# chaofengc/FeMaSR

Measured on AMD Instinct MI355X. Metric: SR output megapixels/sec at x4 (128->512), higher is better.
Workload: dtype f32 (1x1 convs / nn.Linear: every fp32 operand split EXACTLY into three bf16 terms, six partial products, fp32 accumulation on the bf16 matrix pipe - closer to fp64 than the fp32 fmaf chain, bit-identical to the CPU oracle)

## Files before the change

femasr_amd/_lib.py:

```python
import ctypes
import os

_HERE = os.path.dirname(os.path.abspath(__file__))
SO_PATH = os.path.join(_HERE, 'csrc', 'libfemasr_hip.so')

c_int, c_i64, c_f32 = ctypes.c_int, ctypes.c_int64, ctypes.c_float
vp, szt = ctypes.c_void_p, ctypes.c_size_t


class FemasrError(RuntimeError):
    pass


MAX_CODEBOOKS = 3


class Config(ctypes.Structure):
    _fields_ = ([(n, ctypes.c_int32) for n in ('in_channel', 'gt_resolution', 'lq_stage', 'scale_factor', 'use_quantize',
                                               'use_residual', 'n_codebooks')] +
                [(n, ctypes.c_int32 * MAX_CODEBOOKS) for n in ('codebook_scale', 'n_e', 'e_dim')] +
                [('device', ctypes.c_int32)])


class ConvArgs(ctypes.Structure):
# ... 119 lines not shown
    'femasr_channels_merge_u8': (c_int, [vp, vp, vp, vp, c_int, c_int, c_int, c_int, vp, vp, c_int, vp, vp, c_int, vp]),
    'femasr_clock_probe': (c_int, [vp, c_int, vp]),
    'femasr_clock_probe_entries': (c_int, []),
}
ENCODE_SIGNATURES = {
    'femasr_encode_workspace_bytes': (c_int, [vp, c_int, c_int, c_int, c_int, ctypes.POINTER(szt)]),
    'femasr_encode': (c_int, [vp, vp, vp, c_int, c_int, c_int, c_int, c_int, c_int, vp, vp, szt]),
    'femasr_index_histogram_workspace_bytes': (c_int, [c_int, c_i64, c_int, ctypes.POINTER(szt)]),
    'femasr_index_histogram': (c_int, [vp, vp, c_int, c_i64, c_int, vp, vp, vp, szt]),
}
RESAMPLE_SIGNATURES = {
    'femasr_resample_u8': (c_int, [vp, vp, c_int, c_int, c_int, vp, c_int, c_int, vp, vp, c_int, vp, vp, c_int]),
    'femasr_resample_tile': (c_int, []),
}
JPEG_SIGNATURES = {
    'femasr_jpeg_coefficients_u8': (c_int, [vp, c_int, c_int, c_int, c_int, vp, vp, vp, vp, vp, vp]),
    'femasr_jpeg_entropy_rows': (ctypes.c_longlong, [vp, vp, vp, c_int, c_int, c_int, c_int, c_int, c_int, vp, szt]),
    'femasr_jpeg_entropy_bound': (szt, [c_int, c_int, c_int, c_int]),
}
c_u64 = ctypes.c_uint64
DEGRADE_SIGNATURES = {
    'femasr_degrade_blur_f32': (c_int, [vp, vp, c_int, c_int, vp, c_int, c_int, vp]),
    'femasr_degrade_resize_f32': (c_int, [vp, vp, c_int, c_int, vp, c_int, c_int, vp, vp, c_int, vp, vp, c_int, vp, vp]),
    'femasr_degrade_noise_f32': (c_int, [vp, vp, vp, ctypes.c_longlong, c_u64, c_int, ctypes.POINTER(ctypes.c_double), c_u64]),
    'femasr_degrade_quantize_u8': (c_int, [vp, vp, vp, ctypes.c_longlong]),
    'femasr_degrade_unit_f32': (c_int, [vp, vp, c_int, c_int, c_int, vp]),
    'femasr_jpeg_decode_u8': (c_int, [vp, vp, vp, vp, c_int, c_int, c_int, c_int, vp, vp, vp, c_int]),
}
DEBUG_SIGNATURES = {
    'femasr_debug_set_wino_limits': (c_int, [vp, c_int, c_int]),
    'femasr_debug_mfma_bf16': (c_int, [vp, vp, vp, vp, c_int, vp]),
    'femasr_gemm_force_config': (c_int, [c_int]),
    'femasr_conv_small_launch_blocks': (c_int, [c_int]),
    'femasr_debug_conv_variant_name': (c_int, [ctypes.POINTER(ConvArgs), ctypes.c_char_p, c_int]),
    'femasr_debug_weight_image_bytes': (c_int, [vp, c_int, ctypes.POINTER(szt)]),
    'femasr_debug_math_eval': (c_int, [vp, c_int, vp, ctypes.c_longlong, vp]),
}

_lib = None


def load():
    global _lib
    if _lib is not None:
        return _lib
    if not os.path.exists(SO_PATH):
        raise FemasrError(
            f'{SO_PATH} not found: the HIP extension is not built. Run `python femasr_amd/csrc/build.py` '
            '(needs hipcc; cross-compiles gfx950 without a GPU). There is no CPU fallback.')
    lib = ctypes.CDLL(SO_PATH)
    lib.femasr_version.restype = c_int
    if lib.femasr_version() != ABI_VERSION:
        raise FemasrError(f'{SO_PATH} reports ABI version {lib.femasr_version()}, this binding is written for {ABI_VERSION} '
                          '(femasr_conv_args layout): rebuild with `python femasr_amd/csrc/build.py --force`')
    for name, (res, args) in list(SIGNATURES.items()) + list(ENCODE_SIGNATURES.items()) + list(RESAMPLE_SIGNATURES.items()) + list(JPEG_SIGNATURES.items()) + list(DEGRADE_SIGNATURES.items()) + list(DEBUG_SIGNATURES.items()):
        fn = getattr(lib, name)
        fn.restype = res
        fn.argtypes = args
    _lib = lib
    return lib


def check(rc):
    if rc != 0:
        msg = load().femasr_last_error()
        raise FemasrError(f'libfemasr_hip error {rc}: {msg.decode() if msg else "?"}')
# ... 5 lines not shown
```

femasr_amd/csrc/gemm_common.h:

```cpp
#pragma once
#include "conv_common.h"
#include "detmath.h"
#include <stdlib.h>

typedef float f32x16 __attribute__((ext_vector_type(16)));

namespace {

struct GemmParams {
    const float *A;
    const void *W;
    const float *bias, *res1, *res2;
    float *out;
    int M, N, K, MB, NB, NT32;
};

struct GemmFrame {
    int t, lane, wave, wm, wn;
    int nb, mb, m0, n0;
    int h, c31;

    __device__ __forceinline__ GemmFrame(int MB, int NB, int bt)
    {
        t = threadIdx.x, lane = t & 63;
        wave = __builtin_amdgcn_readfirstlane(t >> 6);
        wm = wave >> 1, wn = wave & 1;
        const int L = xcd_remap(blockIdx.x, MB * NB);
        nb = L % NB, mb = L / NB;
        m0 = mb * bt, n0 = nb * bt;
        h = lane >> 5, c31 = lane & 31;
    }
};

template <int WT, int ACT, int NRES, bool NULL_BIAS, class Elem>
__device__ __forceinline__ void gemm_store_epilogue(const GemmParams &p, const GemmFrame &f, float *lds, Elem elem)
{
    const int m0 = f.m0, n0 = f.n0, wm = f.wm, wn = f.wn, h = f.h, c31 = f.c31;
    float *T = lds + f.wave * TSCRATCH;
    const int trow = f.lane >> 3, tq = f.lane & 7;
    const float *ra = p.res1 ? p.res1 : p.res2, *rb = (p.res1 && p.res2) ? p.res2 : nullptr;
    const bool vec = (p.N & 3) == 0;
    f32x4_t r1[4] = {}, r2[4] = {};
    auto fetch_bias = [&](int j) {
        const int col = n0 + (wn * WT + j) * 32 + 4 * tq;
        f32x4_t b4 = {0.f, 0.f, 0.f, 0.f};
        if (!NULL_BIAS || p.bias) b4 = *reinterpret_cast<const f32x4_t *>(p.bias + (col < p.N ? col : 0));
        return b4;
    };
    auto fetch_res = [&](int tl) {
        if (NRES == 0 || !vec) return;
        const int rbase = m0 + (wm * WT + tl / WT) * 32, col = n0 + (wn * WT + tl % WT) * 32 + 4 * tq;
#pragma unroll
        for (int k = 0; k < 4; ++k) {
            const int row = rbase + trow + 8 * k;
            const size_t o = (col < p.N && row < p.M) ? (size_t)row * p.N + col : 0;
            r1[k] = *reinterpret_cast<const f32x4_t *>(ra + o);
            if (NRES >= 2) r2[k] = *reinterpret_cast<const f32x4_t *>(rb + o);
        }
    };
#pragma unroll
    for (int tl = 0; tl < WT * WT; ++tl) {
        const int i = tl / WT, j = tl % WT;
        const int rbase = m0 + (wm * WT + i) * 32, cbase = n0 + (wn * WT + j) * 32;
// ... 41 lines not shown
struct FragItem {
    int lane, n, k0;
    size_t tile;
};
__device__ __forceinline__ FragItem frag_item(size_t item, int NT32)
{
    const int lane = (int)(item & 63);
    const size_t tile = item >> 6;
    const int nt = (int)(tile % NT32), st = (int)(tile / NT32);
    return {lane, 32 * nt + (lane & 31), 16 * st + 8 * (lane >> 5), tile};
}

template <class Params>
struct GemmVariant {
    const char *name;
    void (*kern)(const Params);
    int lds;
    unsigned long long attr_devs;
};

inline int gemm_params(const femasr_conv_args *a, const char *who, int Ho, int Wo, int K, GemmParams &p)
{
    FEMASR_REQUIRE(a->act == FEMASR_ACT_NONE || a->act == FEMASR_ACT_GELU, "%s: bad activation %d", who, a->act);
    const long long M = (long long)a->B * Ho * Wo;
    FEMASR_REQUIRE(a->Ho == Ho && a->Wo == Wo, "%s: Ho/Wo mismatch", who);
    FEMASR_REQUIRE(M > 0 && M < (1ll << 31) - 256, "%s: bad row count", who);
    p.A = a->in; p.bias = a->bias; p.res1 = a->res1; p.res2 = a->res2; p.out = a->out;
    p.M = (int)M; p.N = a->Cout; p.K = K;
    p.NT32 = (p.N + 31) / 32;
    return FEMASR_OK;
}

template <class Params, int N>
int gemm_variant_launch(hipStream_t s, GemmVariant<Params> (&table)[N], int vi, int bt, Params &p, int *variant_out, double *flops_out)
{
    GemmVariant<Params> &v = table[vi];
    p.MB = (p.M + bt - 1) / bt; p.NB = (p.N + bt - 1) / bt;
    FEMASR_CHECK(femasr_allow_dynamic_lds((const void *)v.kern, &v.attr_devs, (size_t)v.lds));
    hipLaunchKernelGGL(v.kern, dim3((unsigned)(p.MB * p.NB)), dim3(256), (size_t)v.lds, s, p);
    FEMASR_CHECK_HIP(hipGetLastError());
    if (variant_out) *variant_out = vi;
    if (flops_out) *flops_out = 2.0 * (double)p.M * (double)p.N * (double)p.K;
    return FEMASR_OK;
}

}
```

femasr_amd/csrc/kernel_meta.py:

```python
import functools
import os
import re
import struct
import subprocess
import sys
import tempfile

HERE = os.path.dirname(os.path.abspath(__file__))
READELF = '/opt/rocm/lib/llvm/bin/llvm-readelf'
ALLOW_SCRATCH = (
    'conv3x3_halo_bf16x3_kernel',
)


def device_elf(obj_path):
    data = open(obj_path, 'rb').read()
    i = data.find(b'__CLANG_OFFLOAD_BUNDLE__')
    if i < 0:
        return None
    n = struct.unpack_from('<Q', data, i + 24)[0]
    off = i + 32
    for _ in range(n):
        o, sz, tl = struct.unpack_from('<QQQ', data, off)
        off += 24
# ... 97 lines not shown
    for line in txt.splitlines():
        m = re.match(r'^[0-9a-f]+ <(\S+)>:', line)
        if m:
            cur = out.setdefault(m.group(1), [])
            continue
        m = re.match(r'^\s+(\S+)\s*(.*?)\s*//\s*([0-9A-Fa-f]+):', line)
        if m and cur is not None:
            cur.append((int(m.group(3), 16), m.group(1), m.group(2)))
    return out


def mfma_loops(insts):
    addr_index = {a: i for i, (a, _, _) in enumerate(insts)}
    loops = []
    for i, (a, op, args) in enumerate(insts):
        if not op.startswith('s_cbranch') and op != 's_branch':
            continue
        try:
            simm = int(args.split()[0])
        except (ValueError, IndexError):
            continue
        if simm >= 32768:
            simm -= 65536
        if simm >= 0:
            continue
        tgt = addr_index.get(a + 4 + 4 * simm)
        if tgt is None:
            continue
        if any(o.startswith('v_mfma') for _, o, _ in insts[tgt:i]):
            loops.append((tgt, i))
    return [l for l in loops if not any(m != l and l[0] <= m[0] and m[1] <= l[1] for m in loops)]


def check_counted_waits(obj=None):
    obj = obj or os.path.join(HERE, 'kernels_gemm_bf16.o')
    problems = []
    src = open(os.path.join(HERE, 'kernels_gemm_bf16.hip')).read()
    src_counts = sorted({int(v) for v in re.findall(r's_waitcnt vmcnt\((\d+)\)', src)})
    want_counts = sorted({0} | set(COUNTED['vmcnt']))
    if src_counts != want_counts:
        problems.append(f'kernels_gemm_bf16.hip waits for vmcnt {src_counts}, kernel_meta.COUNTED expects {want_counts}: update both together')
    seen = 0
    for name, insts in disassemble(obj).items():
        if 'gemm_bf16s_kernel' not in name:
            continue
        seen += 1
        want = COUNTED
        loops = mfma_loops(insts)
        if len(loops) != want['loops']:
            problems.append(f'{demangle_short(name)}: expected {want["loops"]} MFMA loop(s), found {len(loops)}')
            continue
        for lo, hi in loops:
            body = insts[lo:hi + 1]
            vmem, waits = {}, {}
            for _, op, args in body:
                if op.startswith(VMEM_PREFIXES):
                    vmem[op] = vmem.get(op, 0) + 1
                if op == 's_waitcnt':
                    for n in re.findall(r'vmcnt\((\d+)\)', args):
                        waits[int(n)] = waits.get(int(n), 0) + 1
            want_vmem = {k: v for k, v in want.items() if k not in ('vmcnt', 'loops')}
            if vmem != want_vmem:
                problems.append(f'{demangle_short(name)}: VMEM instructions in the MFMA loop {vmem}, the counted waits assume exactly {want_vmem}')
            if waits != want['vmcnt']:
                problems.append(f'{demangle_short(name)}: vmcnt waits in the MFMA loop {waits}, the source has {want["vmcnt"]}')
            if not any(op == 's_barrier' for _, op, _ in body):
                problems.append(f'{demangle_short(name)}: no s_barrier in the MFMA loop')
    if seen < N_GEMM_BF16S:
        problems.append(f'only {seen} gemm_bf16s_kernel instantiations found in {obj}')
    return problems


META = ('vgpr_count', 'agpr_count', 'sgpr_count', 'vgpr_spill_count', 'sgpr_spill_count', 'private_segment_fixed_size', 'group_segment_fixed_size')


def code_of(csrc, objs=None):
    meta = {(r['file'], r['name']): tuple(r.get(k) for k in META) for r in kernels(csrc) if objs is None or r['file'] in objs}
    return {f: {n: ([i[1:] for i in insts], meta[f, n]) for n, insts in disassemble(os.path.join(csrc, f)).items() if (f, n) in meta}
            for f in sorted({f for f, _ in meta})}


def diff(here, there, rename=()):
    ren = dict(rename)
    old = {f: {ren.get(n, n): v for n, v in ks.items()} for f, ks in there.items()}
    lines = [(f, n, 'same' if v == old[f][n] else 'differs') for f, ks in here.items() for n, v in ks.items() if n in old.get(f, {})]
    lone_here = [(f, n) for f, ks in here.items() for n in ks if n not in old.get(f, {})]
    lone_there = [(g, n) for g, ks in old.items() for n in ks if n not in here.get(g, {})]
    for f, n in lone_here:
        homes = [g for g, m in lone_there if m == n]
        if len(homes) == 1:
            lone_there.remove((homes[0], n))
            lines.append((f + ' < ' + homes[0], n, 'same' if here[f][n] == old[homes[0]][n] else 'differs'))
        else:
            lines.append((f, n, 'only here'))
    return sorted(lines + [(g, n, 'only there') for g, n in lone_there])


LOOP_PREFIXES = VMEM_PREFIXES + ('ds_', 'v_mfma', 's_waitcnt', 's_barrier')


# ... 41 lines not shown
```

femasr_amd/csrc/kernels_gemm_bf16.hip:

```cpp
#include "gemm_common.h"

typedef __bf16 bf16x8 __attribute__((ext_vector_type(8)));
typedef __bf16 bf16x2_t __attribute__((ext_vector_type(2)));
typedef float f32x2_t __attribute__((ext_vector_type(2)));

namespace {

struct GemmSParams : GemmParams {
    int imH, imW, Cin, tapmul;
    int imHo, imWo, stride;
};

__device__ float g_gs_zero_page[64];

constexpr int GS_A_HALF = 3 * 2 * 128;
constexpr int GS_A_BYTES = 2 * GS_A_HALF * 16;
constexpr int GS_W_STAGE = 4 * 3 * 64;
constexpr int GS_W_STAGES = 4;
constexpr int GS_LDS_BYTES = GS_A_BYTES + GS_W_STAGES * GS_W_STAGE * 16;
static_assert(4 * TSCRATCH * 4 <= GS_LDS_BYTES, "epilogue scratch overlays the main-loop buffers");

__device__ __forceinline__ unsigned cvt_pk_bf16(float a, float b)
{
    const bf16x2_t r = __builtin_convertvector(f32x2_t{a, b}, bf16x2_t);
    return __builtin_bit_cast(unsigned, r);
}

__device__ __forceinline__ void split3_pair(float a, float b, unsigned &p1, unsigned &p2, unsigned &p3)
{
    p1 = cvt_pk_bf16(a, b);
    const float ra = a - __uint_as_float(p1 << 16), rb = b - __uint_as_float(p1 & 0xffff0000u);
    p2 = cvt_pk_bf16(ra, rb);
    const float sa = ra - __uint_as_float(p2 << 16), sb = rb - __uint_as_float(p2 & 0xffff0000u);
    p3 = cvt_pk_bf16(sa, sb);
}
__device__ __forceinline__ void split3_x8(const f32x4_t &u, const f32x4_t &v, uint4 &q1, uint4 &q2, uint4 &q3)
{
    split3_pair(u[0], u[1], q1.x, q2.x, q3.x);
    split3_pair(u[2], u[3], q1.y, q2.y, q3.y);
    split3_pair(v[0], v[1], q1.z, q2.z, q3.z);
    split3_pair(v[2], v[3], q1.w, q2.w, q3.w);
}

typedef __attribute__((address_space(3))) void *lds_vptr_s;

__device__ __forceinline__ void dma3(const uint4 *w, unsigned d0)
{
    unsigned m0_keep;
    asm volatile("s_mov_b32 %0, m0\n\t"
                 "s_mov_b32 m0, %1\n\ts_nop 0\n\tglobal_load_lds_dwordx4 %4, off\n\t"
                 "s_mov_b32 m0, %2\n\ts_nop 0\n\tglobal_load_lds_dwordx4 %5, off\n\t"
                 "s_mov_b32 m0, %3\n\ts_nop 0\n\tglobal_load_lds_dwordx4 %6, off\n\t"
                 "s_mov_b32 m0, %0"
                 : "=&s"(m0_keep) : "s"(d0), "s"(d0 + 1024u), "s"(d0 + 2048u), "v"(w), "v"(w + 64), "v"(w + 128) : "memory");
}

template <int ACT, int NRES, int CONV>
__global__ __launch_bounds__(256, 2) void gemm_bf16s_kernel(const GemmSParams p)
{
    extern __shared__ __attribute__((aligned(16))) unsigned char smem_raw[];
    uint4 *S = reinterpret_cast<uint4 *>(smem_raw);

    const GemmFrame f(p.MB, p.NB, 128);
    const int t = f.t, lane = f.lane, wave = f.wave, wm = f.wm, wn = f.wn, m0 = f.m0, n0 = f.n0, h = f.h, c31 = f.c31;
    const int nsteps = p.K >> 4;

    int ntile = (n0 >> 5) + wave;
    ntile = ntile < p.NT32 ? ntile : p.NT32 - 1;
    const uint4 *srcW = static_cast<const uint4 *>(p.W) + (size_t)ntile * 192 + lane;
    const size_t wstep = (size_t)p.NT32 * 192;
    const unsigned lds0 = __builtin_amdgcn_readfirstlane((unsigned)(size_t)(lds_vptr_s)S);

    f32x16 hi[2][2], lo[2][2];
#pragma unroll
    for (int i = 0; i < 2; ++i)
#pragma unroll
        for (int j = 0; j < 2; ++j)
#pragma unroll
            for (int r = 0; r < 16; ++r) { hi[i][j][r] = 0.f; lo[i][j][r] = 0.f; }

    auto compute = [&](const uint4 *As, const int (&aoff)[2], const uint4 *Ws) {
        bf16x8 fa[3][2], fb[3][2];
        constexpr int order[3] = {2, 0, 1};
#pragma unroll
        for (int q = 0; q < 3; ++q) {
            const int pa = order[q], pb = q == 0 ? 0 : (q == 1 ? 2 : 1);
#pragma unroll
            for (int rt = 0; rt < 2; ++rt) fa[pa][rt] = __builtin_bit_cast(bf16x8, As[pa * 256 + aoff[rt]]);
#pragma unroll
            for (int ct = 0; ct < 2; ++ct) fb[pb][ct] = __builtin_bit_cast(bf16x8, Ws[ct * 192 + pb * 64]);
        }
#define GS_TERM(ACC, PA, PB)                                                                                       \
    _Pragma("unroll") for (int rt = 0; rt < 2; ++rt)                                                              \
        _Pragma("unroll") for (int ct = 0; ct < 2; ++ct)                                                          \
            ACC[rt][ct] = __builtin_amdgcn_mfma_f32_32x32x16_bf16(fa[PA][rt], fb[PB][ct], ACC[rt][ct], 0, 0, 0);
        GS_TERM(lo, 2, 0)
        GS_TERM(lo, 0, 2)
        GS_TERM(lo, 1, 1)
        GS_TERM(lo, 1, 0)
        GS_TERM(lo, 0, 1)
        GS_TERM(hi, 0, 0)
#undef GS_TERM
    };
    const int boff = (wn * 2) * 192 + lane;

    {
        uint4 *Al = S;
        uint4 *Wl = reinterpret_cast<uint4 *>(smem_raw + GS_A_BYTES);
        const int g2 = t & 1, srow = t >> 1;
        int grow = m0 + srow;
        grow = grow < p.M ? grow : p.M - 1;
        const float *srcA = p.A + (size_t)grow * p.K + 8 * g2;
        unsigned tapmask = 0;
        if (CONV) {
            const int ox = grow % p.imWo, oy = (grow / p.imWo) % p.imHo, n = grow / (p.imWo * p.imHo);
            const int px = ox * p.stride, py = oy * p.stride;
            srcA = p.A + (((size_t)n * p.imH + py) * p.imW + px) * p.Cin + 8 * g2;
#pragma unroll
            for (int tp = 0; tp < 9; ++tp) {
                const int yy = py + tp / 3 - 1, xx = px + tp % 3 - 1;
                tapmask |= (yy >= 0 && yy < p.imH && xx >= 0 && xx < p.imW ? 1u : 0u) << tp;
            }
        }
        const int cpc = p.Cin >> 5;
        const int dstA = g2 * 128 + ((srow + 4 * g2) & 127);
        f32x4_t ar[2][4] = {};
        const int nch = p.K >> 5;
        auto loadA = [&](int c, f32x4_t (&r)[4]) {
            const int cl = c < nch ? c : nch - 1;
            const float *q;
            if (CONV) {
                const int tap = (cl * p.tapmul) >> 20, cc = cl - tap * cpc;
                const int ky = (tap * 11) >> 5, kx = tap - 3 * ky;
                const int off = ((ky - 1) * p.imW + (kx - 1)) * p.Cin + cc * 32;
                q = ((tapmask >> tap) & 1u) ? srcA + off : g_gs_zero_page + 8 * g2;
            } else {
                q = srcA + cl * 32;
            }
            asm volatile("global_load_dwordx4 %0, %4, off\n\tglobal_load_dwordx4 %1, %4, off offset:16\n\t"
                         "global_load_dwordx4 %2, %4, off offset:64\n\tglobal_load_dwordx4 %3, %4, off offset:80"
                         : "=&v"(r[0]), "=&v"(r[1]), "=&v"(r[2]), "=&v"(r[3]) : "v"(q) : "memory");
        };
        const unsigned ldsW = lds0 + (unsigned)GS_A_BYTES + (unsigned)wave * 3072u;
        auto issueW = [&](int s) {
            dma3(srcW + (size_t)(s < nsteps ? s : nsteps - 1) * wstep, ldsW + (unsigned)(s & (GS_W_STAGES - 1)) * (GS_W_STAGE * 16));
        };
        auto splitA = [&](const f32x4_t &u, const f32x4_t &v, int half) {
            uint4 q1, q2, q3;
            split3_x8(u, v, q1, q2, q3);
            uint4 *d = Al + half * GS_A_HALF + dstA;
            d[0] = q1;
            d[256] = q2;
            d[512] = q3;
        };
        int aoff[2];
#pragma unroll
        for (int rt = 0; rt < 2; ++rt) {
            const int row = wm * 64 + rt * 32 + c31;
            aoff[rt] = h * 128 + ((row + 4 * h) & 127);
        }
        auto step = [&](int s) { compute(Al + (s & 1) * GS_A_HALF, aoff, Wl + (s & (GS_W_STAGES - 1)) * GS_W_STAGE + boff); };
        issueW(0);
        loadA(0, ar[0]);
        issueW(1);
        issueW(2);
        loadA(1, ar[1]);
        asm volatile("s_waitcnt vmcnt(10)" : "+v"(ar[0][0]), "+v"(ar[0][1]), "+v"(ar[0][2]), "+v"(ar[0][3]) :: "memory");
        splitA(ar[0][0], ar[0][1], 0);

        auto chunk = [&](int c, f32x4_t (&cur)[4], f32x4_t (&nxt)[4]) {
            asm volatile("s_waitcnt vmcnt(14)\n\ts_waitcnt lgkmcnt(0)" ::: "memory");
            __builtin_amdgcn_s_barrier();
            asm volatile("" ::: "memory");
            issueW(2 * c + 3);
            splitA(cur[2], cur[3], 1);
            step(2 * c);
            asm volatile("s_waitcnt vmcnt(10)\n\ts_waitcnt lgkmcnt(0)" ::: "memory");
            __builtin_amdgcn_s_barrier();
            asm volatile("" ::: "memory");
            issueW(2 * c + 4);
            loadA(c + 2, cur);
            asm volatile("s_waitcnt vmcnt(10)" : "+v"(nxt[0]), "+v"(nxt[1]), "+v"(nxt[2]), "+v"(nxt[3]) :: "memory");
            splitA(nxt[0], nxt[1], 0);
            step(2 * c + 1);
        };
#pragma unroll 1
        for (int c = 0; c < nch; c += 2) {
            chunk(c, ar[0], ar[1]);
            chunk(c + 1, ar[1], ar[0]);
        }
    }

    asm volatile("s_waitcnt vmcnt(0)" ::: "memory");
    float *T = reinterpret_cast<float *>(smem_raw) + wave * TSCRATCH;
    {
        const int trow = lane >> 3, tq = lane & 7;
        const float *ra = p.res1 ? p.res1 : p.res2, *rb = (p.res1 && p.res2) ? p.res2 : nullptr;
        const bool vec = (p.N & 3) == 0;
        f32x4_t bpre[2] = {}, r1[2][4] = {}, r2[2][4] = {};
        auto fetch_res = [&](int tl, f32x4_t (&d1)[4], f32x4_t (&d2)[4]) {
            if (NRES == 0 || !vec) return;
            const int rbase = m0 + (wm * 2 + (tl >> 1)) * 32, col = n0 + (wn * 2 + (tl & 1)) * 32 + 4 * tq;
#pragma unroll
            for (int k = 0; k < 4; ++k) {
                const int row = rbase + trow + 8 * k;
                const size_t o = (col < p.N && row < p.M) ? (size_t)row * p.N + col : 0;
                d1[k] = *reinterpret_cast<const f32x4_t *>(ra + o);
                if (NRES >= 2) d2[k] = *reinterpret_cast<const f32x4_t *>(rb + o);
            }
        };
        if (vec) {
#pragma unroll
            for (int j = 0; j < 2; ++j) {
                const int col = n0 + (wn * 2 + j) * 32 + 4 * tq;
                bpre[j] = *reinterpret_cast<const f32x4_t *>(p.bias + (col < p.N ? col : 0));
            }
        }
        fetch_res(0, r1[0], r2[0]);
        asm volatile("s_waitcnt lgkmcnt(0)" ::: "memory");
        __builtin_amdgcn_s_barrier();
        asm volatile("" ::: "memory");
#pragma unroll
        for (int tl = 0; tl < 4; ++tl) {
            const int i = tl >> 1, j = tl & 1;
            const int rbase = m0 + (wm * 2 + i) * 32, cbase = n0 + (wn * 2 + j) * 32;
            if (vec) {
                const int col = cbase + 4 * tq;
                const bool cok = col < p.N;
                if (tl + 1 < 4) fetch_res(tl + 1, r1[(tl + 1) & 1], r2[(tl + 1) & 1]);
#pragma unroll
                for (int r = 0; r < 16; ++r) T[((r & 3) + 8 * (r >> 2) + 4 * h) * TPITCH + c31] = hi[i][j][r] + lo[i][j][r];
                const f32x4_t b4 = bpre[j];
#pragma unroll
                for (int k = 0; k < 4; ++k) {
                    const f32x4_t a4 = *reinterpret_cast<const f32x4_t *>(T + (trow + 8 * k) * TPITCH + 4 * tq);
                    float v[4] = {a4[0] + b4[0], a4[1] + b4[1], a4[2] + b4[2], a4[3] + b4[3]};
                    if (ACT == FEMASR_ACT_GELU) {
                        const det_f32x2 g0 = det_gelu2(det_f32x2{v[0], v[1]}), g1 = det_gelu2(det_f32x2{v[2], v[3]});
                        v[0] = g0[0]; v[1] = g0[1]; v[2] = g1[0]; v[3] = g1[1];
                    }
#pragma unroll
                    for (int e = 0; e < 4; ++e) {
                        if (NRES >= 1) v[e] = v[e] + r1[tl & 1][k][e];
                        if (NRES >= 2) v[e] = v[e] + r2[tl & 1][k][e];
                    }
                    const int row = rbase + trow + 8 * k;
                    if (cok && row < p.M) *reinterpret_cast<f32x4_t *>(p.out + (size_t)row * p.N + col) = f32x4_t{v[0], v[1], v[2], v[3]};
                }
            } else {
                const int col = cbase + c31;
#pragma unroll
                for (int r = 0; r < 16; ++r) {
                    const int row = rbase + (r & 3) + 8 * (r >> 2) + 4 * h;
                    if (row < p.M && col < p.N) {
                        const size_t o = (size_t)row * p.N + col;
                        float v = (hi[i][j][r] + lo[i][j][r]) + p.bias[col];
                        if (ACT == FEMASR_ACT_GELU) v = det_gelu(v);
                        if (NRES >= 1) v = v + ra[o];
                        if (NRES >= 2) v = v + rb[o];
                        p.out[o] = v;
                    }
                }
            }
        }
    }
}

struct GatherOI {
    static __device__ __forceinline__ void load(const float *in, int I, int n, int k0, f32x4_t &u, f32x4_t &v)
    {
        u = *reinterpret_cast<const f32x4_t *>(in + (size_t)n * I + k0);
        v = *reinterpret_cast<const f32x4_t *>(in + (size_t)n * I + k0 + 4);
    }
};
struct GatherOIHW3x3 {
    static __device__ __forceinline__ void load(const float *in, int I, int n, int k0, f32x4_t &u, f32x4_t &v)
    {
        const int tap = k0 / I, c0 = k0 - tap * I;
        float w[8];
#pragma unroll
        for (int j = 0; j < 8; ++j) w[j] = in[((size_t)n * I + c0 + j) * 9 + tap];
        u = f32x4_t{w[0], w[1], w[2], w[3]};
        v = f32x4_t{w[4], w[5], w[6], w[7]};
    }
};
template <class GATHER>
__global__ void repack_bf16s_kernel(const float *__restrict__ in, int O, int I, uint4 *__restrict__ out, size_t total)
{
    const int NT32 = (O + 31) / 32;
    for (size_t i = blockIdx.x * (size_t)blockDim.x + threadIdx.x; i < total; i += (size_t)gridDim.x * blockDim.x) {
        const FragItem it = frag_item(i, NT32);
        f32x4_t u = {0.f, 0.f, 0.f, 0.f}, v = {0.f, 0.f, 0.f, 0.f};
        if (it.n < O) GATHER::load(in, I, it.n, it.k0, u, v);
        uint4 q1, q2, q3;
        split3_x8(u, v, q1, q2, q3);
        uint4 *o = out + it.tile * 192 + it.lane;
        o[0] = q1;
        o[64] = q2;
        o[128] = q3;
    }
}

__global__ void mfma_bf16_probe_kernel(const unsigned short *__restrict__ a, const unsigned short *__restrict__ b, const float *__restrict__ c,
                                       int N, float *__restrict__ d)
{
    const int lane = threadIdx.x, i = lane & 31, h = lane >> 5;
    const int n = blockIdx.x * 32 + i;
    union { bf16x8 v; unsigned short u[8]; } fa, fb;
#pragma unroll
    for (int e = 0; e < 8; ++e) { fa.u[e] = n < N ? a[(size_t)n * 16 + 8 * h + e] : 0; fb.u[e] = n < N ? b[(size_t)n * 16 + 8 * h + e] : 0; }
    f32x16 acc;
#pragma unroll
    for (int r = 0; r < 16; ++r) acc[r] = ((r & 3) + 8 * (r >> 2) + 4 * h == i && n < N) ? c[n] : 0.f;
    acc = __builtin_amdgcn_mfma_f32_32x32x16_bf16(fa.v, fb.v, acc, 0, 0, 0);
#pragma unroll
    for (int r = 0; r < 16; ++r)
        if ((r & 3) + 8 * (r >> 2) + 4 * h == i && n < N) d[n] = acc[r];
}

#define GS_VARIANT(ACT, NRES) { "gemm_bf16s<act=" #ACT ",nres=" #NRES ">", gemm_bf16s_kernel<ACT, NRES, 0>, GS_LDS_BYTES, 0ull }
#define GC_VARIANT(NRES) { "conv3x3_bf16s<128px x128,9Cin split GEMM,nres=" #NRES ">", gemm_bf16s_kernel<0, NRES, 1>, GS_LDS_BYTES, 0ull }
GemmVariant<GemmSParams> g_gsv[] = { GS_VARIANT(0, 0), GS_VARIANT(0, 1), GS_VARIANT(0, 2), GS_VARIANT(1, 0), GS_VARIANT(1, 1), GS_VARIANT(1, 2),
                      GC_VARIANT(0), GC_VARIANT(1), GC_VARIANT(2) };
constexpr int kNumGS = sizeof(g_gsv) / sizeof(g_gsv[0]);

}

extern "C" size_t femasr_packed_weight_bf16s_bytes(int O, int I) { return (size_t)(I / 16) * ((O + 31) / 32) * 192 * sizeof(uint4); }
bool femasr_gemm_bf16s_shape_ok(const femasr_conv_args *a)
{
    if (a->up2 || (a->Cin % 64) != 0 || a->prologue != FEMASR_PRO_NONE) return false;
    return (a->ksz == 1 && a->pad == 0 && a->stride == 1) || femasr_conv3x3_bf16s_shape_ok(a);
}
bool femasr_conv3x3_bf16s_shape_ok(const femasr_conv_args *a)
{
    return a->ksz == 3 && (a->stride == 1 || a->stride == 2) && a->pad == 1 && !a->up2 && (a->Cin % 64) == 0 && a->Cin <= 1024 && a->prologue == FEMASR_PRO_NONE &&
           a->act == FEMASR_ACT_NONE && (long long)a->B * a->H * a->W * a->Cin < (1ll << 31);
}
int femasr_gemm_bf16s_variant_count() { return kNumGS; }
const char *femasr_gemm_bf16s_variant_name(int v) { return (v >= 0 && v < kNumGS) ? g_gsv[v].name : "?"; }

template <class GATHER>
static int repack_bf16s(void *stream, const float *in, int O, int I, int K, void *out)
{
    const size_t total = (size_t)(K / 16) * ((O + 31) / 32) * 64;
    hipLaunchKernelGGL(repack_bf16s_kernel<GATHER>, dim3(grid_for(total)), dim3(256), 0, (hipStream_t)stream, in, O, I, (uint4 *)out, total);
    FEMASR_CHECK_HIP(hipGetLastError());
    return FEMASR_OK;
}

extern "C" int femasr_repack_k1_bf16s(void *stream, const float *in, int O, int I, void *out)
{
    FEMASR_REQUIRE(in && out && O > 0 && I > 0 && (I % 64) == 0, "repack_k1_bf16s: bad args");
    return repack_bf16s<GatherOI>(stream, in, O, I, I, out);
}

extern "C" size_t femasr_packed_weight_conv3x3_bf16s_bytes(int O, int I) { return femasr_packed_weight_bf16s_bytes(O, 9 * I); }
extern "C" int femasr_repack_oihw_bf16s(void *stream, const float *in, int O, int I, void *out)
{
    FEMASR_REQUIRE(in && out && O > 0 && I > 0 && (I % 64) == 0, "repack_oihw_bf16s: needs a 3x3 OIHW weight with I %% 64 == 0");
    return repack_bf16s<GatherOIHW3x3>(stream, in, O, I, 9 * I, out);
}

extern "C" int femasr_debug_mfma_bf16(void *stream, const uint16_t *a, const uint16_t *b, const float *c, int n, float *d)
{
    FEMASR_REQUIRE(a && b && c && d && n > 0, "debug_mfma_bf16: bad args");
    hipLaunchKernelGGL(mfma_bf16_probe_kernel, dim3((unsigned)((n + 31) / 32)), dim3(64), 0, (hipStream_t)stream, a, b, c, n, d);
    FEMASR_CHECK_HIP(hipGetLastError());
    return FEMASR_OK;
}

int femasr_gemm_bf16s_pick_variant(const femasr_conv_args *a)
{
    const int nres = (a->res1 ? 1 : 0) + (a->res2 ? 1 : 0), act = a->act == FEMASR_ACT_GELU ? 1 : 0;
    return a->ksz == 3 ? 6 + nres : 3 * act + nres;
}

int femasr_gemm_bf16s_launch(hipStream_t s, const femasr_conv_args *a, const void *w_bf16s, int *variant_out, double *flops_out)
{
    FEMASR_REQUIRE(a && a->in && w_bf16s && femasr_gemm_bf16s_shape_ok(a), "gemm_bf16s: layer is neither a 1x1 / linear layer nor a 3x3 pad-1 conv of stride 1 or 2 with Cin %% 64 == 0");
    FEMASR_REQUIRE(a->bias && a->out, "gemm_bf16s: bias/out must be set");
    const bool conv = a->ksz == 3;
    const int Ho = conv ? (a->H - 1) / a->stride + 1 : a->H, Wo = conv ? (a->W - 1) / a->stride + 1 : a->W;
    GemmSParams p{};
    FEMASR_CHECK(gemm_params(a, "gemm_bf16s", Ho, Wo, conv ? 9 * a->Cin : a->Cin, p));
    p.W = w_bf16s;
    p.imH = a->H; p.imW = a->W; p.imHo = Ho; p.imWo = Wo; p.stride = a->stride; p.Cin = a->Cin; p.tapmul = ((1 << 20) + (a->Cin >> 5) - 1) / (a->Cin >> 5);
    return gemm_variant_launch(s, g_gsv, femasr_gemm_bf16s_pick_variant(a), 128, p, variant_out, flops_out);
}
```

include/femasr_hip_debug.h:

```cpp
#ifndef FEMASR_HIP_DEBUG_H
#define FEMASR_HIP_DEBUG_H
#include "femasr_hip.h"
#ifdef __cplusplus
extern "C" {
#endif

int femasr_debug_set_wino_limits(femasr_handle *h, int log2_total, int log2_image);

int femasr_debug_mfma_bf16(void *stream, const uint16_t *a, const uint16_t *b, const float *c, int n, float *d);

int femasr_gemm_force_config(int cfg);
int femasr_conv_small_launch_blocks(int blocks);

int femasr_debug_conv_variant_name(const femasr_conv_args *a, char *name, int cap);

int femasr_debug_weight_image_bytes(const femasr_handle *h, int form, size_t *bytes);

int femasr_debug_math_eval(void *stream, int fn, const float *x, long long n, float *y);

#ifdef __cplusplus
}
#endif
#endif
```

Measured before the change: 67.87.

## Make split-bf16 GEMM persistent and prefetch next tile's loads during current tile

```diff
diff --git a/femasr_amd/_lib.py b/femasr_amd/_lib.py
--- a/femasr_amd/_lib.py
+++ b/femasr_amd/_lib.py
@@ -175,6 +175,7 @@
     'femasr_debug_mfma_bf16': (c_int, [vp, vp, vp, vp, c_int, vp]),
     'femasr_gemm_force_config': (c_int, [c_int]),
     'femasr_conv_small_launch_blocks': (c_int, [c_int]),
+    'femasr_gemm_bf16s_grid_cap': (c_int, [c_int]),
     'femasr_debug_conv_variant_name': (c_int, [ctypes.POINTER(ConvArgs), ctypes.c_char_p, c_int]),
     'femasr_debug_weight_image_bytes': (c_int, [vp, c_int, ctypes.POINTER(szt)]),
     'femasr_debug_math_eval': (c_int, [vp, c_int, vp, ctypes.c_longlong, vp]),
diff --git a/femasr_amd/csrc/gemm_common.h b/femasr_amd/csrc/gemm_common.h
--- a/femasr_amd/csrc/gemm_common.h
+++ b/femasr_amd/csrc/gemm_common.h
@@ -25,10 +25,14 @@
         t = threadIdx.x, lane = t & 63;
         wave = __builtin_amdgcn_readfirstlane(t >> 6);
         wm = wave >> 1, wn = wave & 1;
-        const int L = xcd_remap(blockIdx.x, MB * NB);
+        seat(blockIdx.x, MB, NB, bt);
+        h = lane >> 5, c31 = lane & 31;
+    }
+    __device__ __forceinline__ void seat(int tile, int MB, int NB, int bt)
+    {
+        const int L = xcd_remap(tile, MB * NB);
         nb = L % NB, mb = L / NB;
         m0 = mb * bt, n0 = nb * bt;
-        h = lane >> 5, c31 = lane & 31;
     }
 };
 
@@ -136,12 +140,13 @@
 }
 
 template <class Params, int N>
-int gemm_variant_launch(hipStream_t s, GemmVariant<Params> (&table)[N], int vi, int bt, Params &p, int *variant_out, double *flops_out)
+int gemm_variant_launch(hipStream_t s, GemmVariant<Params> (&table)[N], int vi, int bt, Params &p, int *variant_out, double *flops_out, int max_blocks = 0)
 {
     GemmVariant<Params> &v = table[vi];
     p.MB = (p.M + bt - 1) / bt; p.NB = (p.N + bt - 1) / bt;
     FEMASR_CHECK(femasr_allow_dynamic_lds((const void *)v.kern, &v.attr_devs, (size_t)v.lds));
-    hipLaunchKernelGGL(v.kern, dim3((unsigned)(p.MB * p.NB)), dim3(256), (size_t)v.lds, s, p);
+    const int tiles = p.MB * p.NB;
+    hipLaunchKernelGGL(v.kern, dim3((unsigned)(max_blocks > 0 && max_blocks < tiles ? max_blocks : tiles)), dim3(256), (size_t)v.lds, s, p);
     FEMASR_CHECK_HIP(hipGetLastError());
     if (variant_out) *variant_out = vi;
     if (flops_out) *flops_out = 2.0 * (double)p.M * (double)p.N * (double)p.K;
diff --git a/femasr_amd/csrc/kernel_meta.py b/femasr_amd/csrc/kernel_meta.py
--- a/femasr_amd/csrc/kernel_meta.py
+++ b/femasr_amd/csrc/kernel_meta.py
@@ -153,6 +153,25 @@
     return [l for l in loops if not any(m != l and l[0] <= m[0] and m[1] <= l[1] for m in loops)]
 
 
+def branch_target(insts, i, addr_index):
+    a, op, args = insts[i]
+    if not op.startswith('s_cbranch') and op != 's_branch':
+        return None
+    try:
+        simm = int(args.split()[0])
+    except (ValueError, IndexError):
+        return None
+    if simm >= 32768:
+        simm -= 65536
+    return addr_index.get(a + 4 + 4 * simm)
+
+
+def tile_loop_head(insts, lo, hi):
+    addr_index = {a: i for i, (a, _, _) in enumerate(insts)}
+    heads = [t for t in (branch_target(insts, i, addr_index) for i in range(hi + 1, len(insts))) if t is not None and t < lo]
+    return min(heads) if heads else None
+
+
 def check_counted_waits(obj=None):
     obj = obj or os.path.join(HERE, 'kernels_gemm_bf16.o')
     problems = []
@@ -187,6 +206,13 @@
                 problems.append(f'{demangle_short(name)}: vmcnt waits in the MFMA loop {waits}, the source has {want["vmcnt"]}')
             if not any(op == 's_barrier' for _, op, _ in body):
                 problems.append(f'{demangle_short(name)}: no s_barrier in the MFMA loop')
+            head = tile_loop_head(insts, lo, hi)
+            if head is None:
+                problems.append(f'{demangle_short(name)}: the MFMA loop is not inside a tile loop')
+            else:
+                stray = [args for _, op, args in insts[head:lo] if op == 's_waitcnt' and 'vmcnt' in args]
+                if stray:
+                    problems.append(f'{demangle_short(name)}: vmcnt waits between the head of the tile loop and the MFMA loop: {stray}')
     if seen < N_GEMM_BF16S:
         problems.append(f'only {seen} gemm_bf16s_kernel instantiations found in {obj}')
     return problems
diff --git a/femasr_amd/csrc/kernels_gemm_bf16.hip b/femasr_amd/csrc/kernels_gemm_bf16.hip
--- a/femasr_amd/csrc/kernels_gemm_bf16.hip
+++ b/femasr_amd/csrc/kernels_gemm_bf16.hip
@@ -1,4 +1,5 @@
 #include "gemm_common.h"
+#include <atomic>
 
 typedef __bf16 bf16x8 __attribute__((ext_vector_type(8)));
 typedef __bf16 bf16x2_t __attribute__((ext_vector_type(2)));
@@ -14,11 +15,13 @@
 __device__ float g_gs_zero_page[64];
 
 constexpr int GS_A_HALF = 3 * 2 * 128;
-constexpr int GS_A_BYTES = 2 * GS_A_HALF * 16;
 constexpr int GS_W_STAGE = 4 * 3 * 64;
 constexpr int GS_W_STAGES = 4;
-constexpr int GS_LDS_BYTES = GS_A_BYTES + GS_W_STAGES * GS_W_STAGE * 16;
-static_assert(4 * TSCRATCH * 4 <= GS_LDS_BYTES, "epilogue scratch overlays the main-loop buffers");
+constexpr int GS_W_OFF = GS_A_HALF * 16;
+constexpr int GS_A1_OFF = GS_W_OFF + GS_W_STAGES * GS_W_STAGE * 16;
+constexpr int GS_EPI_OFF = GS_W_OFF + (GS_W_STAGES - 1) * GS_W_STAGE * 16;
+constexpr int GS_LDS_BYTES = GS_A1_OFF + GS_A_HALF * 16;
+static_assert(GS_EPI_OFF + 4 * TSCRATCH * 4 <= GS_LDS_BYTES, "epilogue scratch overlays W stage 3 and A half 1 only");
 
 __device__ __forceinline__ unsigned cvt_pk_bf16(float a, float b)
 {
@@ -61,23 +64,16 @@
     extern __shared__ __attribute__((aligned(16))) unsigned char smem_raw[];
     uint4 *S = reinterpret_cast<uint4 *>(smem_raw);
 
-    const GemmFrame f(p.MB, p.NB, 128);
-    const int t = f.t, lane = f.lane, wave = f.wave, wm = f.wm, wn = f.wn, m0 = f.m0, n0 = f.n0, h = f.h, c31 = f.c31;
+    GemmFrame f(p.MB, p.NB, 128);
+    const int t = f.t, lane = f.lane, wave = f.wave, wm = f.wm, wn = f.wn, h = f.h, c31 = f.c31;
     const int nsteps = p.K >> 4;
-
-    int ntile = (n0 >> 5) + wave;
-    ntile = ntile < p.NT32 ? ntile : p.NT32 - 1;
-    const uint4 *srcW = static_cast<const uint4 *>(p.W) + (size_t)ntile * 192 + lane;
+    const int ntiles = p.MB * p.NB;
+
+    const uint4 *Wlane = static_cast<const uint4 *>(p.W) + lane;
     const size_t wstep = (size_t)p.NT32 * 192;
     const unsigned lds0 = __builtin_amdgcn_readfirstlane((unsigned)(size_t)(lds_vptr_s)S);
 
     f32x16 hi[2][2], lo[2][2];
-#pragma unroll
-    for (int i = 0; i < 2; ++i)
-#pragma unroll
-        for (int j = 0; j < 2; ++j)
-#pragma unroll
-            for (int r = 0; r < 16; ++r) { hi[i][j][r] = 0.f; lo[i][j][r] = 0.f; }
 
     auto compute = [&](const uint4 *As, const int (&aoff)[2], const uint4 *Ws) {
         bf16x8 fa[3][2], fb[3][2];
@@ -104,165 +100,215 @@
     };
     const int boff = (wn * 2) * 192 + lane;
 
-    {
-        uint4 *Al = S;
-        uint4 *Wl = reinterpret_cast<uint4 *>(smem_raw + GS_A_BYTES);
-        const int g2 = t & 1, srow = t >> 1;
+    uint4 *Al = S;
+    uint4 *Wl = reinterpret_cast<uint4 *>(smem_raw + GS_W_OFF);
+    constexpr int A_HALF_STRIDE = GS_A1_OFF / 16;
+    const int g2 = t & 1, srow = t >> 1;
+    struct TileSrc {
+        const float *srcA;
+        unsigned tapmask;
+        int wtile;
+    };
+    auto source = [&](int m0, int n0) {
+        TileSrc ts;
+        int ntile = (n0 >> 5) + wave;
+        ts.wtile = ntile < p.NT32 ? ntile : p.NT32 - 1;
         int grow = m0 + srow;
         grow = grow < p.M ? grow : p.M - 1;
-        const float *srcA = p.A + (size_t)grow * p.K + 8 * g2;
-        unsigned tapmask = 0;
+        ts.srcA = p.A + (size_t)grow * p.K + 8 * g2;
+        ts.tapmask = 0;
         if (CONV) {
             const int ox = grow % p.imWo, oy = (grow / p.imWo) % p.imHo, n = grow / (p.imWo * p.imHo);
             const int px = ox * p.stride, py = oy * p.stride;
-            srcA = p.A + (((size_t)n * p.imH + py) * p.imW + px) * p.Cin + 8 * g2;
+            ts.srcA = p.A + (((size_t)n * p.imH + py) * p.imW + px) * p.Cin + 8 * g2;
 #pragma unroll
             for (int tp = 0; tp < 9; ++tp) {
                 const int yy = py + tp / 3 - 1, xx = px + tp % 3 - 1;
-                tapmask |= (yy >= 0 && yy < p.imH && xx >= 0 && xx < p.imW ? 1u : 0u) << tp;
+                ts.tapmask |= (yy >= 0 && yy < p.imH && xx >= 0 && xx < p.imW ? 1u : 0u) << tp;
             }
         }
-        const int cpc = p.Cin >> 5;
-        const int dstA = g2 * 128 + ((srow + 4 * g2) & 127);
-        f32x4_t ar[2][4] = {};
-        const int nch = p.K >> 5;
-        auto loadA = [&](int c, f32x4_t (&r)[4]) {
-            const int cl = c < nch ? c : nch - 1;
-            const float *q;
-            if (CONV) {
-                const int tap = (cl * p.tapmul) >> 20, cc = cl - tap * cpc;
-                const int ky = (tap * 11) >> 5, kx = tap - 3 * ky;
-                const int off = ((ky - 1) * p.imW + (kx - 1)) * p.Cin + cc * 32;
-                q = ((tapmask >> tap) & 1u) ? srcA + off : g_gs_zero_page + 8 * g2;
-            } else {
-                q = srcA + cl * 32;
-            }
-            asm volatile("global_load_dwordx4 %0, %4, off\n\tglobal_load_dwordx4 %1, %4, off offset:16\n\t"
-                         "global_load_dwordx4 %2, %4, off offset:64\n\tglobal_load_dwordx4 %3, %4, off offset:80"
-                         : "=&v"(r[0]), "=&v"(r[1]), "=&v"(r[2]), "=&v"(r[3]) : "v"(q) : "memory");
-        };
-        const unsigned ldsW = lds0 + (unsigned)GS_A_BYTES + (unsigned)wave * 3072u;
-        auto issueW = [&](int s) {
-            dma3(srcW + (size_t)(s < nsteps ? s : nsteps - 1) * wstep, ldsW + (unsigned)(s & (GS_W_STAGES - 1)) * (GS_W_STAGE * 16));
-        };
-        auto splitA = [&](const f32x4_t &u, const f32x4_t &v, int half) {
-            uint4 q1, q2, q3;
-            split3_x8(u, v, q1, q2, q3);
-            uint4 *d = Al + half * GS_A_HALF + dstA;
-            d[0] = q1;
-            d[256] = q2;
-            d[512] = q3;
-        };
-        int aoff[2];
-#pragma unroll
-        for (int rt = 0; rt < 2; ++rt) {
-            const int row = wm * 64 + rt * 32 + c31;
-            aoff[rt] = h * 128 + ((row + 4 * h) & 127);
-        }
-        auto step = [&](int s) { compute(Al + (s & 1) * GS_A_HALF, aoff, Wl + (s & (GS_W_STAGES - 1)) * GS_W_STAGE + boff); };
-        issueW(0);
-        loadA(0, ar[0]);
-        issueW(1);
-        issueW(2);
-        loadA(1, ar[1]);
-        asm volatile("s_waitcnt vmcnt(10)" : "+v"(ar[0][0]), "+v"(ar[0][1]), "+v"(ar[0][2]), "+v"(ar[0][3]) :: "memory");
-        splitA(ar[0][0], ar[0][1], 0);
-
-        auto chunk = [&](int c, f32x4_t (&cur)[4], f32x4_t (&nxt)[4]) {
-            asm volatile("s_waitcnt vmcnt(14)\n\ts_waitcnt lgkmcnt(0)" ::: "memory");
-            __builtin_amdgcn_s_barrier();
-            asm volatile("" ::: "memory");
-            issueW(2 * c + 3);
-            splitA(cur[2], cur[3], 1);
-            step(2 * c);
-            asm volatile("s_waitcnt vmcnt(10)\n\ts_waitcnt lgkmcnt(0)" ::: "memory");
-            __builtin_amdgcn_s_barrier();
-            asm volatile("" ::: "memory");
-            issueW(2 * c + 4);
-            loadA(c + 2, cur);
-            asm volatile("s_waitcnt vmcnt(10)" : "+v"(nxt[0]), "+v"(nxt[1]), "+v"(nxt[2]), "+v"(nxt[3]) :: "memory");
-            splitA(nxt[0], nxt[1], 0);
-            step(2 * c + 1);
-        };
+        return ts;
+    };
+    TileSrc here = source(f.m0, f.n0), ahead = here;
+    const int cpc = p.Cin >> 5;
+    const int dstA = g2 * 128 + ((srow + 4 * g2) & 127);
+    f32x4_t ar[2][4] = {};
+    const int nch = p.K >> 5;
+    auto loadA = [&](int c, f32x4_t (&r)[4]) {
+        const bool own = c < nch;
+        const int cl = own ? c : c - nch;
+        const float *base = own ? here.srcA : ahead.srcA;
+        const float *q;
+        if (CONV) {
+            const unsigned tapmask = own ? here.tapmask : ahead.tapmask;
+            const int tap = (cl * p.tapmul) >> 20, cc = cl - tap * cpc;
+            const int ky = (tap * 11) >> 5, kx = tap - 3 * ky;
+            const int off = ((ky - 1) * p.imW + (kx - 1)) * p.Cin + cc * 32;
+            q = ((tapmask >> tap) & 1u) ? base + off : g_gs_zero_page + 8 * g2;
+        } else {
+            q = base + cl * 32;
+        }
+        asm volatile("global_load_dwordx4 %0, %4, off\n\tglobal_load_dwordx4 %1, %4, off offset:16\n\t"
+                     "global_load_dwordx4 %2, %4, off offset:64\n\tglobal_load_dwordx4 %3, %4, off offset:80"
+                     : "=&v"(r[0]), "=&v"(r[1]), "=&v"(r[2]), "=&v"(r[3]) : "v"(q) : "memory");
+    };
+    const unsigned ldsW = lds0 + (unsigned)GS_W_OFF + (unsigned)wave * 3072u;
+    auto issueW = [&](int s) {
+        const size_t off = s < nsteps ? (size_t)here.wtile * 192 + (size_t)s * wstep : (size_t)ahead.wtile * 192 + (size_t)(s - nsteps) * wstep;
+        dma3(Wlane + off, ldsW + (unsigned)(s & (GS_W_STAGES - 1)) * (GS_W_STAGE * 16));
+    };
+    auto splitA = [&](const f32x4_t &u, const f32x4_t &v, int half) {
+        uint4 q1, q2, q3;
+        split3_x8(u, v, q1, q2, q3);
+        uint4 *d = Al + half * A_HALF_STRIDE + dstA;
+        d[0] = q1;
+        d[256] = q2;
+        d[512] = q3;
+    };
+    int aoff[2];
+#pragma unroll
+    for (int rt = 0; rt < 2; ++rt) {
+        const int row = wm * 64 + rt * 32 + c31;
+        aoff[rt] = h * 128 + ((row + 4 * h) & 127);
+    }
+    auto step = [&](int s) { compute(Al + (s & 1) * A_HALF_STRIDE, aoff, Wl + (s & (GS_W_STAGES - 1)) * GS_W_STAGE + boff); };
+    issueW(0);
+    loadA(0, ar[0]);
+    issueW(1);
+    issueW(2);
+    loadA(1, ar[1]);
+    asm volatile("s_waitcnt vmcnt(10)" : "+v"(ar[0][0]), "+v"(ar[0][1]), "+v"(ar[0][2]), "+v"(ar[0][3]) :: "memory");
+    splitA(ar[0][0], ar[0][1], 0);
+
+    auto chunk = [&](int c, f32x4_t (&cur)[4], f32x4_t (&nxt)[4]) {
+        asm volatile("s_waitcnt vmcnt(14)\n\ts_waitcnt lgkmcnt(0)" ::: "memory");
+        __builtin_amdgcn_s_barrier();
+        asm volatile("" ::: "memory");
+        issueW(2 * c + 3);
+        splitA(cur[2], cur[3], 1);
+        step(2 * c);
+        asm volatile("s_waitcnt vmcnt(10)\n\ts_waitcnt lgkmcnt(0)" ::: "memory");
+        __builtin_amdgcn_s_barrier();
+        asm volatile("" ::: "memory");
+        issueW(2 * c + 4);
+        loadA(c + 2, cur);
+        asm volatile("s_waitcnt vmcnt(10)" : "+v"(nxt[0]), "+v"(nxt[1]), "+v"(nxt[2]), "+v"(nxt[3]) :: "memory");
+        splitA(nxt[0], nxt[1], 0);
+        step(2 * c + 1);
+    };
+#pragma unroll 1
+    for (int tile = blockIdx.x;;) {
+        const int m0 = f.m0, n0 = f.n0;
+        const int tnext = tile + (int)gridDim.x;
+        const bool more = tnext < ntiles;
+        if (more) {
+            f.seat(tnext, p.MB, p.NB, 128);
+            ahead = source(f.m0, f.n0);
+        } else {
+            ahead = here;
+        }
+#pragma unroll
+        for (int i = 0; i < 2; ++i)
+#pragma unroll
+            for (int j = 0; j < 2; ++j)
+#pragma unroll
+                for (int r = 0; r < 16; ++r) { hi[i][j][r] = 0.f; lo[i][j][r] = 0.f; }
 #pragma unroll 1
         for (int c = 0; c < nch; c += 2) {
             chunk(c, ar[0], ar[1]);
             chunk(c + 1, ar[1], ar[0]);
         }
-    }
-
-    asm volatile("s_waitcnt vmcnt(0)" ::: "memory");
-    float *T = reinterpret_cast<float *>(smem_raw) + wave * TSCRATCH;
-    {
-        const int trow = lane >> 3, tq = lane & 7;
-        const float *ra = p.res1 ? p.res1 : p.res2, *rb = (p.res1 && p.res2) ? p.res2 : nullptr;
-        const bool vec = (p.N & 3) == 0;
-        f32x4_t bpre[2] = {}, r1[2][4] = {}, r2[2][4] = {};
-        auto fetch_res = [&](int tl, f32x4_t (&d1)[4], f32x4_t (&d2)[4]) {
-            if (NRES == 0 || !vec) return;
-            const int rbase = m0 + (wm * 2 + (tl >> 1)) * 32, col = n0 + (wn * 2 + (tl & 1)) * 32 + 4 * tq;
-#pragma unroll
-            for (int k = 0; k < 4; ++k) {
-                const int row = rbase + trow + 8 * k;
-                const size_t o = (col < p.N && row < p.M) ? (size_t)row * p.N + col : 0;
-                d1[k] = *reinterpret_cast<const f32x4_t *>(ra + o);
-                if (NRES >= 2) d2[k] = *reinterpret_cast<const f32x4_t *>(rb + o);
-            }
-        };
-        if (vec) {
-#pragma unroll
-            for (int j = 0; j < 2; ++j) {
-                const int col = n0 + (wn * 2 + j) * 32 + 4 * tq;
-                bpre[j] = *reinterpret_cast<const f32x4_t *>(p.bias + (col < p.N ? col : 0));
-            }
-        }
-        fetch_res(0, r1[0], r2[0]);
-        asm volatile("s_waitcnt lgkmcnt(0)" ::: "memory");
-        __builtin_amdgcn_s_barrier();
-        asm volatile("" ::: "memory");
-#pragma unroll
-        for (int tl = 0; tl < 4; ++tl) {
-            const int i = tl >> 1, j = tl & 1;
-            const int rbase = m0 + (wm * 2 + i) * 32, cbase = n0 + (wn * 2 + j) * 32;
+
+        asm volatile("s_waitcnt vmcnt(0)" : "+v"(ar[1][0]), "+v"(ar[1][1]), "+v"(ar[1][2]), "+v"(ar[1][3]) :: "memory");
+        float *T = reinterpret_cast<float *>(smem_raw + GS_EPI_OFF) + wave * TSCRATCH;
+        {
+            const int trow = lane >> 3, tq = lane & 7;
+            const float *ra = p.res1 ? p.res1 : p.res2, *rb = (p.res1 && p.res2) ? p.res2 : nullptr;
+            const bool vec = (p.N & 3) == 0;
+            f32x4_t bpre[2] = {}, r1[2][4] = {}, r2[4] = {};
+            auto res_off = [&](int tl, int k) {
+                const int row = m0 + (wm * 2 + (tl >> 1)) * 32 + trow + 8 * k, col = n0 + (wn * 2 + (tl & 1)) * 32 + 4 * tq;
+                return (col < p.N && row < p.M) ? (size_t)row * p.N + col : (size_t)0;
+            };
+            auto fetch_r1 = [&](int tl) {
+                if (NRES == 0) return;
+#pragma unroll
+                for (int k = 0; k < 4; ++k) r1[tl & 1][k] = *reinterpret_cast<const f32x4_t *>(ra + res_off(tl, k));
+            };
+            auto fetch_r2 = [&](int tl) {
+                if (NRES < 2) return;
+#pragma unroll
+                for (int k = 0; k < 4; ++k) r2[k] = *reinterpret_cast<const f32x4_t *>(rb + res_off(tl, k));
+            };
             if (vec) {
-                const int col = cbase + 4 * tq;
-                const bool cok = col < p.N;
-                if (tl + 1 < 4) fetch_res(tl + 1, r1[(tl + 1) & 1], r2[(tl + 1) & 1]);
-#pragma unroll
-                for (int r = 0; r < 16; ++r) T[((r & 3) + 8 * (r >> 2) + 4 * h) * TPITCH + c31] = hi[i][j][r] + lo[i][j][r];
-                const f32x4_t b4 = bpre[j];
-#pragma unroll
-                for (int k = 0; k < 4; ++k) {
-                    const f32x4_t a4 = *reinterpret_cast<const f32x4_t *>(T + (trow + 8 * k) * TPITCH + 4 * tq);
-                    float v[4] = {a4[0] + b4[0], a4[1] + b4[1], a4[2] + b4[2], a4[3] + b4[3]};
-                    if (ACT == FEMASR_ACT_GELU) {
-                        const det_f32x2 g0 = det_gelu2(det_f32x2{v[0], v[1]}), g1 = det_gelu2(det_f32x2{v[2], v[3]});
-                        v[0] = g0[0]; v[1] = g0[1]; v[2] = g1[0]; v[3] = g1[1];
+#pragma unroll
+                for (int j = 0; j < 2; ++j) {
+                    const int col = n0 + (wn * 2 + j) * 32 + 4 * tq;
+                    bpre[j] = *reinterpret_cast<const f32x4_t *>(p.bias + (col < p.N ? col : 0));
+                }
+                fetch_r1(0);
+                fetch_r2(0);
+                asm volatile("s_waitcnt lgkmcnt(0)" ::: "memory");
+                __builtin_amdgcn_s_barrier();
+                asm volatile("" ::: "memory");
+#pragma unroll
+                for (int tl = 0; tl < 4; ++tl) {
+                    const int i = tl >> 1, j = tl & 1;
+                    const int rbase = m0 + (wm * 2 + i) * 32, cbase = n0 + (wn * 2 + j) * 32;
+                    const int col = cbase + 4 * tq;
+                    const bool cok = col < p.N;
+                    if (tl + 1 < 4) fetch_r1(tl + 1);
+#pragma unroll
+                    for (int r = 0; r < 16; ++r) T[((r & 3) + 8 * (r >> 2) + 4 * h) * TPITCH + c31] = hi[i][j][r] + lo[i][j][r];
+                    const f32x4_t b4 = bpre[j];
+#pragma unroll
+                    for (int k = 0; k < 4; ++k) {
+                        const f32x4_t a4 = *reinterpret_cast<const f32x4_t *>(T + (trow + 8 * k) * TPITCH + 4 * tq);
+                        float v[4] = {a4[0] + b4[0], a4[1] + b4[1], a4[2] + b4[2], a4[3] + b4[3]};
+                        if (ACT == FEMASR_ACT_GELU) {
+                            const det_f32x2 g0 = det_gelu2(det_f32x2{v[0], v[1]}), g1 = det_gelu2(det_f32x2{v[2], v[3]});
+                            v[0] = g0[0]; v[1] = g0[1]; v[2] = g1[0]; v[3] = g1[1];
+                        }
+#pragma unroll
+                        for (int e = 0; e < 4; ++e) {
+                            if (NRES >= 1) v[e] = v[e] + r1[tl & 1][k][e];
+                            if (NRES >= 2) v[e] = v[e] + r2[k][e];
+                        }
+                        const int row = rbase + trow + 8 * k;
+                        asm volatile("" :: "v"(bpre[j]));
+                        if (NRES >= 1) asm volatile("" :: "v"(r1[tl & 1][k]));
+                        if (NRES >= 2) asm volatile("" :: "v"(r2[k]));
+                        if (cok && row < p.M) *reinterpret_cast<f32x4_t *>(p.out + (size_t)row * p.N + col) = f32x4_t{v[0], v[1], v[2], v[3]};
                     }
-#pragma unroll
-                    for (int e = 0; e < 4; ++e) {
-                        if (NRES >= 1) v[e] = v[e] + r1[tl & 1][k][e];
-                        if (NRES >= 2) v[e] = v[e] + r2[tl & 1][k][e];
-                    }
-                    const int row = rbase + trow + 8 * k;
-                    if (cok && row < p.M) *reinterpret_cast<f32x4_t *>(p.out + (size_t)row * p.N + col) = f32x4_t{v[0], v[1], v[2], v[3]};
+                    if (tl + 1 < 4) fetch_r2(tl + 1);
                 }
             } else {
-                const int col = cbase + c31;
-#pragma unroll
-                for (int r = 0; r < 16; ++r) {
-                    const int row = rbase + (r & 3) + 8 * (r >> 2) + 4 * h;
-                    if (row < p.M && col < p.N) {
-                        const size_t o = (size_t)row * p.N + col;
-                        float v = (hi[i][j][r] + lo[i][j][r]) + p.bias[col];
-                        if (ACT == FEMASR_ACT_GELU) v = det_gelu(v);
-                        if (NRES >= 1) v = v + ra[o];
-                        if (NRES >= 2) v = v + rb[o];
-                        p.out[o] = v;
+                asm volatile("s_waitcnt lgkmcnt(0)" ::: "memory");
+                __builtin_amdgcn_s_barrier();
+                asm volatile("" ::: "memory");
+#pragma unroll
+                for (int tl = 0; tl < 4; ++tl) {
+                    const int i = tl >> 1, j = tl & 1;
+                    const int rbase = m0 + (wm * 2 + i) * 32, cbase = n0 + (wn * 2 + j) * 32;
+                    const int col = cbase + c31;
+#pragma unroll
+                    for (int r = 0; r < 16; ++r) {
+                        const int row = rbase + (r & 3) + 8 * (r >> 2) + 4 * h;
+                        if (row < p.M && col < p.N) {
+                            const size_t o = (size_t)row * p.N + col;
+                            float v = (hi[i][j][r] + lo[i][j][r]) + p.bias[col];
+                            if (ACT == FEMASR_ACT_GELU) v = det_gelu(v);
+                            if (NRES >= 1) v = v + ra[o];
+                            if (NRES >= 2) v = v + rb[o];
+                            p.out[o] = v;
+                        }
                     }
                 }
             }
         }
+        if (!more) break;
+        here = ahead;
+        tile = tnext;
     }
 }
 
@@ -324,6 +370,21 @@
                       GC_VARIANT(0), GC_VARIANT(1), GC_VARIANT(2) };
 constexpr int kNumGS = sizeof(g_gsv) / sizeof(g_gsv[0]);
 
+std::atomic<int> g_gs_grid_cap{0};
+std::atomic<int> g_gs_cus[64];
+int gs_max_blocks()
+{
+    int dev = 0, cus = 0;
+    if (hipGetDevice(&dev) != hipSuccess || dev < 0 || dev >= 64) dev = -1;
+    if (dev >= 0) cus = g_gs_cus[dev].load(std::memory_order_relaxed);
+    if (cus <= 0) {
+        if (dev < 0 || hipDeviceGetAttribute(&cus, hipDeviceAttributeMultiprocessorCount, dev) != hipSuccess || cus <= 0) cus = 256;
+        if (dev >= 0) g_gs_cus[dev].store(cus, std::memory_order_relaxed);
+    }
+    const int cap = g_gs_grid_cap.load(std::memory_order_relaxed);
+    return cap > 0 && cap < 2 * cus ? cap : 2 * cus;
+}
+
 }
 
 extern "C" size_t femasr_packed_weight_bf16s_bytes(int O, int I) { return (size_t)(I / 16) * ((O + 31) / 32) * 192 * sizeof(uint4); }
@@ -386,5 +447,10 @@
     FEMASR_CHECK(gemm_params(a, "gemm_bf16s", Ho, Wo, conv ? 9 * a->Cin : a->Cin, p));
     p.W = w_bf16s;
     p.imH = a->H; p.imW = a->W; p.imHo = Ho; p.imWo = Wo; p.stride = a->stride; p.Cin = a->Cin; p.tapmul = ((1 << 20) + (a->Cin >> 5) - 1) / (a->Cin >> 5);
-    return gemm_variant_launch(s, g_gsv, femasr_gemm_bf16s_pick_variant(a), 128, p, variant_out, flops_out);
-}
+    return gemm_variant_launch(s, g_gsv, femasr_gemm_bf16s_pick_variant(a), 128, p, variant_out, flops_out, gs_max_blocks());
+}
+
+extern "C" int femasr_gemm_bf16s_grid_cap(int blocks)
+{
+    return g_gs_grid_cap.exchange(blocks > 0 ? blocks : 0, std::memory_order_relaxed);
+}
diff --git a/include/femasr_hip_debug.h b/include/femasr_hip_debug.h
--- a/include/femasr_hip_debug.h
+++ b/include/femasr_hip_debug.h
@@ -11,6 +11,7 @@
 
 int femasr_gemm_force_config(int cfg);
 int femasr_conv_small_launch_blocks(int blocks);
+int femasr_gemm_bf16s_grid_cap(int blocks);
 
 int femasr_debug_conv_variant_name(const femasr_conv_args *a, char *name, int cap);
 
```

Result: no change. 68.32, median of 6 (+0.7%).
